# VinAIResearch/Point-Unet

Hardware: AMD Instinct MI355X
Metric: points_per_sec_forward (higher is better)
Workload: dtype f32

## Files before the change

point-unet_amd/csrc/b3_ops.h:

```cpp
#pragma once

#include <hip/hip_runtime.h>

#include "common.h"
#include "mfma_tile.h"

namespace ps {

__device__ __forceinline__ void b3_split_pair(float x, float y, unsigned& q1, unsigned& q2, unsigned& q3)
{
    const unsigned xu = __float_as_uint(x), yu = __float_as_uint(y);
    const float xr = x - __uint_as_float(xu & 0xffff0000u), yr = y - __uint_as_float(yu & 0xffff0000u);
    const unsigned xru = __float_as_uint(xr), yru = __float_as_uint(yr);
    const float x3 = xr - __uint_as_float(xru & 0xffff0000u), y3 = yr - __uint_as_float(yru & 0xffff0000u);
    q1 = __builtin_amdgcn_perm(yu, xu, 0x07060302u);
    q2 = __builtin_amdgcn_perm(yru, xru, 0x07060302u);
    q3 = __builtin_amdgcn_perm(__float_as_uint(y3), __float_as_uint(x3), 0x07060302u);
}
template <int P>
struct BPlanes {
    uint4 p[P];
};
typedef BPlanes<3> B3Planes;
typedef __bf16 b3_bf16x2 __attribute__((ext_vector_type(2)));
// ... 14 lines not shown
    } else {
        r.p[0].x = b3_rne_pair(lo.x, lo.y);
        r.p[0].y = b3_rne_pair(lo.z, lo.w);
        r.p[0].z = b3_rne_pair(hi.x, hi.y);
        r.p[0].w = b3_rne_pair(hi.z, hi.w);
    }
    return r;
}
template <int P>
__device__ __forceinline__ BPlanes<P> b3_split8(const float (&x)[8])
{
    return b3_split8<P>(make_float4(x[0], x[1], x[2], x[3]), make_float4(x[4], x[5], x[6], x[7]));
}
__device__ __forceinline__ f32x16 b3_mfma(const uint4& a, const uint4& b, f32x16 acc)
{
    return __builtin_amdgcn_mfma_f32_32x32x16_bf16(__builtin_bit_cast(bf16x8, a), __builtin_bit_cast(bf16x8, b), acc, 0, 0, 0);
}
template <int P>
__device__ __forceinline__ f32x16 b3_mfma6(const BPlanes<P>& a, const BPlanes<P>& b, f32x16 acc)
{
    if constexpr (P == 3) {
        acc = b3_mfma(a.p[2], b.p[0], acc);
        acc = b3_mfma(a.p[0], b.p[2], acc);
        acc = b3_mfma(a.p[1], b.p[1], acc);
        acc = b3_mfma(a.p[1], b.p[0], acc);
        acc = b3_mfma(a.p[0], b.p[1], acc);
        acc = b3_mfma(a.p[0], b.p[0], acc);
    } else {
        acc = b3_mfma(a.p[0], b.p[0], acc);
    }
    return acc;
}

inline uint16_t b3_piece_of(float w, int plane)
{
    auto trunc16 = [](float x) {
        uint32_t u;
        __builtin_memcpy(&u, &x, 4);
        u &= 0xffff0000u;
        float r;
        __builtin_memcpy(&r, &u, 4);
        return r;
    };
    volatile float w1 = trunc16(w);
    volatile float r1 = w - w1;
    volatile float w2 = trunc16(r1);
    volatile float w3 = r1 - w2;
    const float pick = plane == 0 ? w1 : (plane == 1 ? w2 : w3);
    uint32_t u;
    __builtin_memcpy(&u, &pick, 4);
    return (uint16_t)(u >> 16);
}

template <int P, bool KMAP>
__device__ __forceinline__ void b3_pack_elem(const PackJob& j, int64_t i)
{
    const int ncb = j.cout / 32;
    const int lane = (int)(i & 63), cb = (int)((i >> 6) % ncb), q = (int)((i >> 6) / ncb);
    const int hl = lane >> 5;
    const float* src = j.w + (int64_t)(32 * cb + (lane & 31)) * j.sn;
    float v[8];
#pragma unroll
    for (int e = 0; e < 8; ++e) {
        const int k = KMAP ? 32 * (q >> 1) + 16 * (q & 1) + 8 * (e >> 2) + 4 * hl + (e & 3) : 16 * q + 8 * hl + e;
        v[e] = src[(int64_t)k * j.sk];
    }
// ... 15 lines not shown
```

point-unet_amd/csrc/common.h:

```cpp
#pragma once

#include <hip/hip_runtime.h>

#include <cstdarg>
#include <cstdint>
#include <cstdio>
#include <cstring>
#include <map>
#include <string>
#include <vector>

#include "../../include/pointseg.h"
#include "../../include/pointseg_train_ops.h"

namespace ps {

void set_error(const char* fmt, ...);

#define PS_HIP(expr)                                                                                  \
    do {                                                                                              \
        hipError_t _e = (expr);                                                                       \
        if (_e != hipSuccess) {                                                                       \
            ps::set_error("%s failed: %s (%s:%d)", #expr, hipGetErrorString(_e), __FILE__, __LINE__); \
            return PS_EHIP;                                                                           \
// ... 90 lines not shown
    bool inv_bucket = true;
    int inv_tile = 4096;
    bool gather_reduce_ordered = true;
    int maxpool_bwd_ordered = 1;
    bool train_act_bf16 = true;
    int train_att_gemm_split = -1;
    bool train_att_gemm = true;
    bool train_att128_fwd_gemm = true;
    bool train_fuse_residual = true;
    bool train_merge_syncbn = true;
    int convbn_max_c = 64;
    int convbn_rect_max = 1 << 30;
    bool wgrad_debug = false;
};
void tuning_from_env(Tuning& t);
}

struct ps_context {
    int device = 0;
    ps::Tuning tune;
    hipStream_t own_stream = nullptr;
    hipStream_t stream = nullptr;
    ps::Arena knn_arena;
    ps::Arena net_arena;
    ps::Arena sample_arena;
    ps::DevBuf stage_in;
    ps::DevBuf stage_out;
    ps::DevBuf red_ws;
    ps::DevBuf wgrad_ws;
    ps::PackCache* pack_cache = nullptr;
    ps::DevBuf ops_ring[4];
    int ops_ring_pos = 0;
    bool att_bf16x3 = true;
    bool train_b3 = true;
    bool conv_w_transposed = false;
    bool att_df_accum = false;
    const int32_t* walk_order = nullptr;
    int64_t walk_order_n = 0;
    bool pool_bwd_overwrite = false;
    bool train_bf16 = false;
    bool train_act_bf16 = false;
    bool mid_lds_attr = false;
    size_t chain_lds_attr = 48 * 1024;
    std::map<const void*, size_t> regchain_lds_attr;
    bool deferred = false;
    int32_t* h_flags = nullptr;
    unsigned pending_mask = 0;
    uint64_t builds = 0;
    uint64_t samples = 0;
    uint64_t volume_samples = 0;
    uint64_t flag_serial[8] = {};
    int flag_kind[8] = {};
    int flag_slot = 0;
    int sticky_rc = 0;
    std::string sticky_msg;
    hipEvent_t flag_ev[8] = {};
    std::vector<char> host_ring[8];
    int ring_pos = 0;
    std::vector<char>& ring_next() { ring_pos = (ring_pos + 1) & 7; return host_ring[ring_pos]; }
    int check_deferred();
    int check_flag_slot(int s);
    int defer_status(const void* d_words, size_t bytes, int kind, uint64_t serial);
    struct PinSlot { void* p = nullptr; size_t cap = 0; hipEvent_t ev = nullptr; bool busy = false; };
    PinSlot pin[16];
    int pin_pos = 0;
    int upload_async(void* dst, const void* src, size_t bytes);
// ... 69 lines not shown
```

point-unet_amd/csrc/context.hip:

```cpp
#include "common.h"
#include "kdtree_build.h"

#include <cstdlib>

namespace ps {

static thread_local char g_err[512] = "";

void set_error(const char* fmt, ...)
{
    va_list ap;
    va_start(ap, fmt);
    vsnprintf(g_err, sizeof g_err, fmt, ap);
    va_end(ap);
}

int DevBuf::reserve(size_t bytes)
{
    if (bytes <= cap) return PS_OK;
    if (p) {
        hipError_t e = hipDeviceSynchronize();
        if (e != hipSuccess) {
            set_error("hipDeviceSynchronize failed: %s", hipGetErrorString(e));
            return PS_EHIP;
// ... 186 lines not shown
    flag("PS_TRAIN_ATT128_FWD_GEMM", t.train_att128_fwd_gemm);
    flag("PS_TRAIN_FUSE_RESIDUAL", t.train_fuse_residual);
    flag("PS_TRAIN_MERGE_SYNCBN", t.train_merge_syncbn);
    if (num("PS_CONVBN_MAX_C", v) && v >= 0 && v <= 4096) t.convbn_max_c = (int)v;
    if (num("PS_CONVBN_RECT_MAX", v) && v >= 0) t.convbn_rect_max = v > (double)(1 << 30) ? 1 << 30 : (int)v;
    t.wgrad_debug = std::getenv("PS_WGRAD_DEBUG") != nullptr;
#else
    (void)t;
#endif
}
}

extern "C" {
const char* ps_version(void) { return "pointseg-hip 0.1 gfx950"; }
int ps_abi_version(void) { return PS_ABI_VERSION; }

int ps_create(int device, ps_context** out)
{
    PS_CHECK(out != nullptr, "ps_create: out is NULL");
    int count = 0;
    PS_HIP(hipGetDeviceCount(&count));
    PS_CHECK(device >= 0 && device < count, "ps_create: device %d out of range (%d devices)", device, count);
    PS_HIP(hipSetDevice(device));
    ps_context* c = new ps_context();
    c->device = device;
    hipError_t e = hipStreamCreateWithFlags(&c->own_stream, hipStreamNonBlocking);
    if (e != hipSuccess) {
        delete c;
        ps::set_error("hipStreamCreate failed: %s", hipGetErrorString(e));
        return PS_EHIP;
    }
    c->stream = c->own_stream;
    ps::tuning_from_env(c->tune);
    *out = c;
    return PS_OK;
}

int ps_destroy(ps_context* c)
{
    if (!c) return PS_OK;
    (void)hipSetDevice(c->device);
    (void)hipStreamSynchronize(c->stream);
    c->knn_arena.buf.release();
    c->net_arena.buf.release();
    c->sample_arena.buf.release();
    c->stage_in.release();
    c->stage_out.release();
    c->red_ws.release();
    c->wgrad_ws.release();
    for (auto& b : c->ops_ring) b.release();
    if (c->h_flags) (void)hipHostFree(c->h_flags);
    for (auto& e : c->flag_ev)
        if (e) (void)hipEventDestroy(e);
    for (auto& s : c->pin) {
        if (s.p) (void)hipHostFree(s.p);
        if (s.ev) (void)hipEventDestroy(s.ev);
    }
    for (hipEvent_t e : c->event_pool) (void)hipEventDestroy(e);
    if (c->own_stream) (void)hipStreamDestroy(c->own_stream);
    delete c;
    return PS_OK;
}

int ps_set_stream(ps_context* c, void* hip_stream)
{
    PS_CHECK(c != nullptr, "ps_set_stream: ctx is NULL");
// ... 94 lines not shown
```

point-unet_amd/csrc/debug_hooks.h:

```cpp
#ifndef POINTSEG_DEBUG_H
#define POINTSEG_DEBUG_H
#include "../../include/pointseg.h"
#ifdef __cplusplus
extern "C" {
#endif
int ps_debug_knn_host(const float* support, const float* queries, int64_t B, int64_t n_support,
                      int64_t n_queries, int64_t K, int32_t* out_idx);
int ps_debug_kdtree_host(const float* support, int64_t n, int32_t* vind, int32_t* nodes, float* pts,
                         int32_t* root_depth, float* bbox);
int ps_debug_kdtree_device(ps_context* ctx, const float* support, int64_t n, int32_t* vind, int32_t* nodes,
                           float* pts, int32_t* root_depth, float* bbox);
#define PS_DEBUG_KDTREE_STATS 22
int ps_debug_kdtree_device_set(ps_context* ctx, const float* support, const int32_t* n, int64_t T, const int32_t* want_copy, int32_t* vind,
                               int32_t* nodes, float* pts, int32_t* fat, int32_t* root_depth, float* bbox, float* copy, int32_t* stats);
int ps_debug_pack_weights(const float* W, int cin, int cout, int ntb, float* out);
int ps_debug_pack_b3(const float* W, int cin, int cout, uint16_t* out);
int ps_debug_gemm32(ps_context* ctx, int split_bf16, const float* x1, int ld1, int c1, const int32_t* g1, const float* x2, int ld2, int c2,
                    const int32_t* g2, int gm, int gn, const float* W, const float* bias, int64_t R, int cout, int leaky, float* y, int ldy);
int ps_debug_gemm32_plan(ps_context* ctx, int split_bf16, int64_t R, int cin, int cout, int* out4);

typedef struct ps_debug_chain_layer {
    const float* W;
    const float* bias;
    int cin, cout, leaky;
    float* y;
    int ldy;
    const float* extra;
    int ld_extra, c_extra;
    const int32_t* extra_gather;
} ps_debug_chain_layer;
typedef struct ps_debug_chain_desc {
    int n_layers;
    ps_debug_chain_layer layer[4];
    const float* x1; const int32_t* g1; int ld1, c1, g1m, g1n;
    const float* x2; const int32_t* g2; int ld2, c2, g2m, g2n;
    int64_t R;
} ps_debug_chain_desc;
int ps_debug_chain(ps_context* ctx, const ps_debug_chain_desc* d, int form);
int ps_debug_chain_plan(const ps_debug_chain_desc* d, int* out4);
int ps_debug_att_stage(ps_randla* net, int level, int stage, int form, const float* xyz, const int32_t* idx, const int32_t* order, const float* fg,
                       int64_t n_total, int64_t n_cloud, float* agg);

int ps_debug_set_tuning(ps_context* ctx, const char* field, double value);
int ps_debug_get_tuning(ps_context* ctx, const char* field, double* value);
int ps_debug_tuning_fields(char* buf, int cap);
int ps_debug_volume_sample_args_size(void);

#ifdef __cplusplus
}
#endif
#endif
```

point-unet_amd/csrc/debug_hooks.hip:

```cpp
#include "common.h"

#include <cstring>
#include <vector>
#include "kdtree_build.h"
#include "kdtree_host.h"
#include "rowgemm.h"
#include "attpool.h"
#include "debug_hooks.h"
#include "randla_net.h"

using namespace ps;

extern "C" int ps_debug_volume_sample_args_size(void) { return (int)sizeof(ps_volume_sample_args); }

extern "C" int ps_debug_pack_weights(const float* W, int cin, int cout, int ntb, float* out)
{
    PS_CHECK(W && out && (ntb == 1 || ntb == 2 || ntb == 4), "ps_debug_pack_weights: bad argument");
    pack_weights(W, cin, cout, ntb, out);
    return PS_OK;
}

extern "C" int ps_debug_pack_b3(const float* W, int cin, int cout, uint16_t* out)
{
    PS_CHECK(W && out && cin > 0 && cin % 32 == 0 && cout > 0 && cout % 32 == 0, "ps_debug_pack_b3: bad argument");
// ... 160 lines not shown
        if (form == 0) {
            ChainCache cache;
            if (rowchain_fits(b.steps, b.n, b.s1, b.s2)) rc = rowchain(c, b.steps, b.n, b.s1, b.s2, d->R, &cache);
            else { set_error("ps_debug_chain: the chain fits neither chain kernel (channels above %d, mismatched, or a gathered extra)", kChainMaxC); rc = PS_EINVAL; }
            (void)hipStreamSynchronize(c->stream);
            cache.clear();
        } else if (form == 1) {
            if (regchain_fits(b.steps, b.n, b.s1, b.s2)) rc = regchain(c, b.steps, b.n, b.s1, b.s2, d->R, nullptr);
            else { set_error("ps_debug_chain: not one of regchain's compiled chain shapes"); rc = PS_EINVAL; }
        } else if (form == 2) {
            if (rowchain_lds_plan(b.steps, b.n, b.s1, b.s2, d->R).form == 2) rc = rowchain_lds(c, b.steps, b.n, b.s1, b.s2, d->R);
            else { set_error("ps_debug_chain: the chain does not fit the LDS-staged kernel (channels above %d, mismatched, or a gathered extra)", kChainMaxC); rc = PS_EINVAL; }
        } else {
            RowSrc in1 = b.s1, in2 = b.s2;
            for (int i = 0; i < b.n && rc == PS_OK; ++i) {
                const ChainStep& st = b.steps[i];
                if (i > 0) {
                    in2 = RowSrc();
                    if (st.extra.x) in2 = st.extra;
                }
                float* out = st.y ? st.y : dev + tmp_off[i];
                const int ldo = st.y ? st.ldy : b.L[i].cout;
                rc = rowgemm(c, b.L[i], in1, in2, d->R, out, ldo);
                in1 = RowSrc();
                in1.x = out; in1.ld = ldo; in1.c = b.L[i].cout;
            }
        }
    }
    (void)hipStreamSynchronize(c->stream);
    (void)hipFree(dev);
    return rc;
}

extern "C" int ps_debug_att_stage(ps_randla* net, int level, int stage, int form, const float* xyz, const int32_t* idx, const int32_t* order,
                                  const float* fg, int64_t n_total, int64_t n_cloud, float* agg)
{
    PS_CHECK(net && xyz && idx && fg && agg, "ps_debug_att_stage: NULL argument");
    PS_CHECK(net->have_weights, "ps_debug_att_stage: weights not set");
    PS_CHECK(level >= 0 && level < net->cfg.num_layers && (stage == 1 || stage == 2) && form >= 0 && form <= 3, "ps_debug_att_stage: bad level / stage / form");
    PS_CHECK(n_total >= 0 && n_cloud >= 1 && n_total % n_cloud == 0, "ps_debug_att_stage: n_total must be a whole number of clouds");
    ps_context* c = net->ctx;
    PS_HIP(hipSetDevice(c->device));
    const EncLevel& e = net->enc[level];
    const int d = e.d, h = d / 2;
    const bool use_g = d >= 64;
    AttStage s;
    s.xyz = xyz; s.idx = idx; s.order = order; s.fg = fg; s.lfa1 = &e.lfa1; s.agg = agg;
    s.n_total = n_total; s.n_cloud = n_cloud; s.d = d; s.k = net->cfg.k_n; s.ldf = use_g ? h + d : h;
    s.p32 = e.has_p32 ? &e.p32 : nullptr;
    s.lfa2 = stage == 2 ? &e.lfa2 : nullptr;
    s.wbot = use_g ? (stage == 1 ? &e.bot1 : &e.bot2) : nullptr;
    s.wfull = use_g ? nullptr : (stage == 1 ? &e.full1 : &e.full2);
    int rc = PS_EINVAL;
    if (form == 0) rc = att_pool_stage(c, s);
    else if (form == 1 && att_pool32b_fits(s)) rc = att_pool32b_stage(c, s);
    else if (form == 2 && att_pool32_fits(s)) rc = att_pool32_stage(c, s);
    else if (form == 3) rc = att_pool16_stage(c, s);
    else set_error("ps_debug_att_stage: the level (d = %d, %lld rows) does not fit the 32x32 form %d", d, (long long)n_total, form);
    (void)hipStreamSynchronize(c->stream);
    return rc;
}

static bool is_bool(double v) { return v == 0 || v == 1; }
static bool is_int_in(double v, double lo, double hi) { return v >= lo && v <= hi && v == (double)(int64_t)v; }

#define PS_TUNING_FIELDS(X)                                                \
// ... 176 lines not shown
```

point-unet_amd/csrc/regchain.hip:

```cpp
#include <algorithm>

#include "mfma_tile.h"
#include "rowgemm.h"

namespace ps {

struct RcLayer {
    const float* wp;
    const float* bias;
    float* y;
    const float* ex;
    int ca, cb;
    int ta, tb;
    int cout, ot;
    int ks, ntb;
    int ldy, ldex, leaky;
    int w_off, b_off;
};
struct RcArgs {
    const float* x1; const int32_t* g1; int ld1, g1m, g1n;
    const float* x2; const int32_t* g2; int ld2, g2m, g2n;
    int n, R;
    RcLayer l[kChainMaxSteps];
    const float* image;
    int image_floats;
};

template <int N_, int A0_, int B0_, int O0_, int B1_ = 0, int O1_ = 0, int B2_ = 0, int O2_ = 0, int B3_ = 0, int O3_ = 0>
struct RcShape {
    static constexpr int N = N_, A0 = A0_;
    static constexpr int B[4] = {B0_, B1_, B2_, B3_};
    static constexpr int O[4] = {O0_, O1_, O2_, O3_};
    static constexpr int A(int l) { return l == 0 ? A0_ : O[l - 1]; }
    static constexpr int IN(int l) { return A(l) + B[l]; }
    static constexpr int maxt()
    {
        int m = 1;
        for (int l = 0; l < N_; ++l) {
            m = IN(l) > m ? IN(l) : m;
            m = O[l] > m ? O[l] : m;
        }
        return m;
    }
};

template <int T0, int NT, int MT>
__device__ __forceinline__ void rc_load(float (&dst)[MT][4], const float* __restrict__ rowp, int c, bool vec, int g)
{
#pragma unroll
    for (int t = 0; t < NT; ++t) {
        const int ch = t * 16 + 4 * g;
        if (vec) {
            float4 v = make_float4(0.f, 0.f, 0.f, 0.f);
            if (t + 1 < NT || ch < c) v = *reinterpret_cast<const float4*>(rowp + ch);
            dst[T0 + t][0] = v.x; dst[T0 + t][1] = v.y; dst[T0 + t][2] = v.z; dst[T0 + t][3] = v.w;
        } else {
#pragma unroll
            for (int q = 0; q < 4; ++q) dst[T0 + t][q] = (t + 1 < NT || ch + q < c) ? rowp[ch + q] : 0.f;
        }
    }
}

template <class S, int L>
__device__ __forceinline__ void rc_layer(const RcArgs& a, float (&act)[S::maxt()][4], const float* lds, int lane, int g, int row, int rr, bool ok)
{
    if constexpr (L < S::N) {
        constexpr int IT = S::IN(L), OT = S::O[L], TA = S::A(L), TB = S::B[L];
        const RcLayer& y = a.l[L];
        if constexpr (L > 0 && TB > 0) {
            const bool ve = (y.cb & 3) == 0 && (y.ldex & 3) == 0 && (reinterpret_cast<uintptr_t>(y.ex) & 15) == 0;
            rc_load<TA, TB>(act, y.ex + (size_t)rr * y.ldex, y.cb, ve, g);
        }
        f32x4 acc[OT];
#pragma unroll
        for (int to = 0; to < OT; ++to) acc[to] = f32x4{0.f, 0.f, 0.f, 0.f};
        if constexpr (L > 0) __builtin_amdgcn_sched_barrier(0);
        const float* w = lds + y.w_off + lane;
#pragma unroll
        for (int t0 = 0; t0 < OT; t0 += 4) {
#pragma unroll
            for (int ti = 0; ti < IT; ++ti)
#pragma unroll
                for (int q = 0; q < 4; ++q)
#pragma unroll
                    for (int to = t0; to < (t0 + 4 < OT ? t0 + 4 : OT); ++to)
                        acc[to] = __builtin_amdgcn_mfma_f32_16x16x4f32(w[((to * IT + ti) * 4 + q) * 64], act[ti][q], acc[to], 0, 0, 0);
            if (t0 + 4 < OT) __builtin_amdgcn_sched_barrier(0);
        }
        const bool vy = y.y && (y.cout & 3) == 0 && (y.ldy & 3) == 0 && (reinterpret_cast<uintptr_t>(y.y) & 15) == 0;
#pragma unroll
        for (int to = 0; to < OT; ++to) {
            const int ch = to * 16 + 4 * g;
            const float4 b = *reinterpret_cast<const float4*>(lds + y.b_off + ch);
            float v[4] = {acc[to][0] + b.x, acc[to][1] + b.y, acc[to][2] + b.z, acc[to][3] + b.w};
#pragma unroll
            for (int q = 0; q < 4; ++q) {
                if (y.leaky) v[q] = leaky02(v[q]);
                act[to][q] = v[q];
            }
            if (y.y && ok) {
                float* o = y.y + (size_t)row * y.ldy + ch;
                if (vy) {
                    if (to + 1 < OT || ch < y.cout) *reinterpret_cast<float4*>(o) = make_float4(v[0], v[1], v[2], v[3]);
                } else {
#pragma unroll
                    for (int q = 0; q < 4; ++q)
                        if (to + 1 < OT || ch + q < y.cout) o[q] = v[q];
                }
            }
        }
        rc_layer<S, L + 1>(a, act, lds, lane, g, row, rr, ok);
    }
}

__device__ __forceinline__ void rc_stage(const RcArgs& a, float* dst)
{
    for (int l = 0; l < a.n; ++l) {
        const RcLayer& y = a.l[l];
        const int it_n = y.ta + y.tb;
        const int ln = threadIdx.x & 63, q = threadIdx.x >> 6;
        const int i = ln & 15, gg = ln >> 4;
        const int npairs = it_n * y.ot;
        for (int base = 0; base < npairs; base += 8) {
            float v[8];
#pragma unroll
            for (int u = 0; u < 8; ++u) {
                const int pr = base + u;
                v[u] = 0.f;
                if (pr < npairs) {
                    const int ti = pr / y.ot, to = pr - ti * y.ot;
                    int k;
                    bool kok;
                    if (ti < y.ta) { k = ti * 16 + 4 * gg + q; kok = k < y.ca; }
                    else { k = (ti - y.ta) * 16 + 4 * gg + q; kok = k < y.cb; k += y.ca; }
                    const int cblk = to / y.ntb, j = to - cblk * y.ntb;
                    if (kok && to * 16 + i < y.cout) v[u] = y.wp[(((size_t)cblk * y.ks + (k >> 2)) * 64 + ((k & 3) * 16 + i)) * y.ntb + j];
                }
            }
#pragma unroll
            for (int u = 0; u < 8; ++u) {
                const int pr = base + u;
                if (pr < npairs) {
                    const int ti = pr / y.ot, to = pr - ti * y.ot;
                    dst[y.w_off + ((to * it_n + ti) * 4 + q) * 64 + ln] = v[u];
                }
            }
        }
        for (int e = threadIdx.x; e < y.ot * 16; e += 256) dst[y.b_off + e] = e < y.cout ? y.bias[e] : 0.f;
    }
}

__global__ __launch_bounds__(256) void rc_pack_kernel(RcArgs a, float* out) { rc_stage(a, out); }

template <class S>
__global__ __launch_bounds__(256) void regchain_kernel(RcArgs a)
{
    extern __shared__ __attribute__((aligned(16))) float rc_lds[];
    constexpr int MT = S::maxt();
    const int wave = threadIdx.x >> 6, lane = threadIdx.x & 63;
    const int p = lane & 15, g = lane >> 4;
    if (a.image) {
        for (int i = threadIdx.x; i < a.image_floats / 4; i += 256) reinterpret_cast<float4*>(rc_lds)[i] = reinterpret_cast<const float4*>(a.image)[i];
    } else {
        rc_stage(a, rc_lds);
    }
    __syncthreads();

    const bool v1 = (a.l[0].ca & 3) == 0 && (a.ld1 & 3) == 0 && (reinterpret_cast<uintptr_t>(a.x1) & 15) == 0;
    const bool v2 = (a.l[0].cb & 3) == 0 && (a.ld2 & 3) == 0 && (reinterpret_cast<uintptr_t>(a.x2) & 15) == 0;
    const int stride = gridDim.x * 4;
    auto load_inputs = [&](int tile, float (&dst)[MT][4]) {
        const int rr = min(tile * 16 + p, a.R - 1);
        const int s1 = a.g1 ? (a.g1m ? (rr / a.g1m) * a.g1n : 0) + a.g1[rr] : rr;
        rc_load<0, S::A0>(dst, a.x1 + (size_t)s1 * a.ld1, a.l[0].ca, v1, g);
        if constexpr (S::B[0] > 0) {
            const int s2 = a.g2 ? (a.g2m ? (rr / a.g2m) * a.g2n : 0) + a.g2[rr] : rr;
            rc_load<S::A0, S::B[0]>(dst, a.x2 + (size_t)s2 * a.ld2, a.l[0].cb, v2, g);
        }
    };
    int tile = blockIdx.x * 4 + wave;
    float act[MT][4], nxt[MT][4];
    if (tile * 16 < a.R) load_inputs(tile, nxt);
    for (; tile * 16 < a.R; tile += stride) {
#pragma unroll
        for (int t = 0; t < S::IN(0); ++t)
#pragma unroll
            for (int q = 0; q < 4; ++q) act[t][q] = nxt[t][q];
        if ((tile + stride) * 16 < a.R) load_inputs(tile + stride, nxt);
        const int row = tile * 16 + p;
        rc_layer<S, 0>(a, act, rc_lds, lane, g, row, min(row, a.R - 1), row < a.R);
    }
}

static inline int rc_tiles(int c) { return (c + 15) / 16; }

using RcFc0 = RcShape<2, 1, 0, 1, 0, 1>;
using RcEnc0 = RcShape<2, 1, 0, 1, 1, 2>;
using RcOne0 = RcShape<1, 1, 0, 1>;
using RcPair1 = RcShape<2, 2, 0, 2, 0, 4>;
using RcPair1b = RcShape<2, 4, 0, 2, 0, 4>;
using RcEnc1 = RcShape<2, 4, 0, 4, 2, 8>;
using RcPair2 = RcShape<2, 8, 0, 4, 0, 8>;
using RcHead = RcShape<4, 2, 2, 2, 0, 4, 0, 2, 0, 1>;

template <class S>
static bool rc_matches(const RcArgs& a)
{
    if (a.n != S::N) return false;
    for (int l = 0; l < S::N; ++l)
        if (a.l[l].ta != S::A(l) || a.l[l].tb != S::B[l] || a.l[l].ot != S::O[l]) return false;
    return true;
}

static bool rc_build(const ChainStep* steps, int n_steps, const RowSrc& s1, const RowSrc& s2, RcArgs& a, size_t& lds_bytes)
{
    if (n_steps < 1 || n_steps > kChainMaxSteps) return false;
    a = RcArgs{};
    a.x1 = s1.x; a.g1 = s1.gather; a.ld1 = s1.ld; a.g1m = s1.gm; a.g1n = s1.gn;
    a.x2 = s2.x; a.g2 = s2.gather; a.ld2 = s2.ld; a.g2m = s2.gm; a.g2n = s2.gn;
    a.n = n_steps;
    int off = 0, prev = 0;
    for (int i = 0; i < n_steps; ++i) {
        const PackedLinear* L = steps[i].L;
        if (!L || !L->wp || !L->bias) return false;
        if (steps[i].extra.x && (i == 0 || steps[i].extra.gather)) return false;
        RcLayer& y = a.l[i];
        y.wp = L->wp; y.bias = L->bias; y.y = steps[i].y; y.ldy = steps[i].ldy;
        y.ex = i > 0 ? steps[i].extra.x : nullptr; y.ldex = steps[i].extra.ld;
        y.ca = i == 0 ? s1.c : prev;
        y.cb = i == 0 ? s2.c : (steps[i].extra.x ? steps[i].extra.c : 0);
        if (y.ca + y.cb != L->cin) return false;
        y.ta = rc_tiles(y.ca); y.tb = rc_tiles(y.cb);
        y.cout = L->cout; y.ot = rc_tiles(L->cout);
        y.ks = L->ks; y.ntb = L->ntb; y.leaky = L->leaky;
        y.w_off = off; off += y.ot * (y.ta + y.tb) * 256;
        y.b_off = off; off += y.ot * 16;
        prev = L->cout;
    }
    lds_bytes = (size_t)off * sizeof(float);
    return rc_matches<RcFc0>(a) || rc_matches<RcEnc0>(a) || rc_matches<RcOne0>(a) || rc_matches<RcPair1>(a) || rc_matches<RcPair1b>(a) ||
           rc_matches<RcEnc1>(a) || rc_matches<RcPair2>(a) || rc_matches<RcHead>(a);
}

bool regchain_fits(const ChainStep* steps, int n_steps, const RowSrc& s1, const RowSrc& s2)
{
    RcArgs a;
    size_t lds = 0;
    return rc_build(steps, n_steps, s1, s2, a, lds);
}

static int rc_blocks(int64_t R, size_t lds_bytes)
{
    const int64_t tiles = (R + 15) / 16;
    const int per_cu = std::max(1, std::min(4, (int)(160 * 1024 / std::max<size_t>(lds_bytes, 1))));
    return (int)std::max<int64_t>(1, std::min<int64_t>((tiles + 3) / 4, 256 * per_cu));
}

ChainPlan regchain_plan(const ChainStep* steps, int n_steps, const RowSrc& s1, const RowSrc& s2, int64_t R)
{
    ChainPlan p;
    RcArgs a;
    if (!rc_build(steps, n_steps, s1, s2, a, p.lds_bytes)) return ChainPlan();
    p.form = 1;
    p.blocks = rc_blocks(R, p.lds_bytes);
    return p;
}

template <class S>
static int rc_launch(ps_context* c, const RcArgs& a, size_t lds_bytes, int blocks)
{
    size_t& have = c->regchain_lds_attr[reinterpret_cast<const void*>(regchain_kernel<S>)];
    if (lds_bytes > 48 * 1024 && lds_bytes > have) {
        PS_HIP(hipFuncSetAttribute(reinterpret_cast<const void*>(regchain_kernel<S>), hipFuncAttributeMaxDynamicSharedMemorySize, (int)lds_bytes));
        have = lds_bytes;
    }
    hipLaunchKernelGGL(regchain_kernel<S>, dim3(blocks), dim3(256), lds_bytes, c->stream, a);
    return PS_OK;
}

int regchain(ps_context* c, const ChainStep* steps, int n_steps, const RowSrc& s1, const RowSrc& s2, int64_t R, ChainCache* cache)
{
    if (R <= 0) return PS_OK;
    RcArgs a;
    size_t lds_bytes = 0;
    PS_CHECK(rc_build(steps, n_steps, s1, s2, a, lds_bytes), "regchain: not one of the compiled chain shapes");
    PS_CHECK(R < (int64_t)1 << 31, "regchain: too many rows");
    a.R = (int)R;
    if (cache) {
        ChainCache::Entry* hit = nullptr;
        for (auto& e : cache->entries)
            if (e.wp0 == a.l[0].wp && e.wp_last == a.l[n_steps - 1].wp && e.n == n_steps && e.ca == a.l[0].ca && e.cb == a.l[0].cb) hit = &e;
        if (!hit) {
            cache->entries.emplace_back();
            hit = &cache->entries.back();
            hit->wp0 = a.l[0].wp; hit->wp_last = a.l[n_steps - 1].wp; hit->n = n_steps; hit->ca = a.l[0].ca; hit->cb = a.l[0].cb;
            PS_TRY(hit->img.reserve(lds_bytes));
            hipLaunchKernelGGL(rc_pack_kernel, dim3(1), dim3(256), 0, c->stream, a, hit->img.as<float>());
            PS_HIP(hipGetLastError());
        }
        a.image = hit->img.as<float>();
        a.image_floats = (int)(lds_bytes / sizeof(float));
    }
    const int blocks = rc_blocks(R, lds_bytes);
    if (rc_matches<RcFc0>(a)) PS_TRY(rc_launch<RcFc0>(c, a, lds_bytes, blocks));
    else if (rc_matches<RcEnc0>(a)) PS_TRY(rc_launch<RcEnc0>(c, a, lds_bytes, blocks));
    else if (rc_matches<RcOne0>(a)) PS_TRY(rc_launch<RcOne0>(c, a, lds_bytes, blocks));
    else if (rc_matches<RcPair1>(a)) PS_TRY(rc_launch<RcPair1>(c, a, lds_bytes, blocks));
    else if (rc_matches<RcPair1b>(a)) PS_TRY(rc_launch<RcPair1b>(c, a, lds_bytes, blocks));
    else if (rc_matches<RcEnc1>(a)) PS_TRY(rc_launch<RcEnc1>(c, a, lds_bytes, blocks));
    else if (rc_matches<RcPair2>(a)) PS_TRY(rc_launch<RcPair2>(c, a, lds_bytes, blocks));
    else PS_TRY(rc_launch<RcHead>(c, a, lds_bytes, blocks));
    PS_HIP(hipGetLastError());
    return PS_OK;
}

}
```

point-unet_amd/csrc/rowgemm.h:

```cpp
#pragma once

#include <vector>

#include "common.h"

namespace ps {

struct PackedLinear {
    const float* wp = nullptr;
    const float* wq = nullptr;
    const void* wb = nullptr;
    const float* w32 = nullptr;
    const void* w32b = nullptr;
    const float* bias = nullptr;
    int cin = 0, cout = 0;
    int ks = 0;
    int ntb = 0;
    int cblocks = 0;
    int leaky = 0;
    int accum = 0;
    size_t packed_floats() const { return (size_t)cblocks * ks * 64 * ntb; }
    int nchunks() const { return (cin + 63) / 64; }
    size_t kperm_floats() const { return (size_t)cblocks * nchunks() * 16 * 64 * ntb; }
    size_t bf16_bytes() const { return (size_t)cblocks * nchunks() * 2 * 64 * ntb * 16; }
// ... 8 lines not shown
struct RowSrc {
    const float* x = nullptr;
    const int32_t* gather = nullptr;
    int ld = 0;
    int c = 0;
    int gm = 0, gn = 0;
};

struct Gemm32Plan {
    int rw = 1, cw = 1, sk = 1, pd = 2;
    int rgroups = 0, cgroups = 0;
};
Gemm32Plan gemm32_plan(const Tuning& tn, int64_t R, int cin, int cout);
Gemm32Plan gemm32b_plan(const Tuning& tn, int64_t R, int cin, int cout);
bool gemm32_fits(const PackedLinear& L, const RowSrc& s1, const RowSrc& s2, int64_t R, int ldy);
int gemm32(ps_context* c, const PackedLinear& L, const RowSrc& s1, const RowSrc& s2, int64_t R, float* y, int ldy);
void pack_p32b(const float* W, int cin, int cout, uint16_t* out);
bool gemm32b_fits(const PackedLinear& L, const RowSrc& s1, const RowSrc& s2, int64_t R, int ldy);
int gemm32b(ps_context* c, const PackedLinear& L, const RowSrc& s1, const RowSrc& s2, int64_t R, float* y, int ldy);

int rowgemm(ps_context* c, const PackedLinear& L, const RowSrc& s1, const RowSrc& s2, int64_t R, float* y, int ldy);

constexpr int kChainMaxC = 96;
constexpr int kChainMaxSteps = 4;
struct ChainStep {
    const PackedLinear* L = nullptr;
    float* y = nullptr;
    int ldy = 0;
    RowSrc extra;
};
bool rowchain_fits(const ChainStep* steps, int n_steps, const RowSrc& s1, const RowSrc& s2);
bool regchain_fits(const ChainStep* steps, int n_steps, const RowSrc& s1, const RowSrc& s2);
struct ChainCache {
    struct Entry { const float* wp0 = nullptr; const float* wp_last = nullptr; int n = 0, ca = 0, cb = 0; DevBuf img; };
    std::vector<Entry> entries;
    void clear()
    {
        for (auto& e : entries) e.img.release();
        entries.clear();
    }
};
int regchain(ps_context* c, const ChainStep* steps, int n_steps, const RowSrc& s1, const RowSrc& s2, int64_t R, ChainCache* cache);
int rowchain_lds(ps_context* c, const ChainStep* steps, int n_steps, const RowSrc& s1, const RowSrc& s2, int64_t R);
struct ChainPlan {
    int form = 0;
    int blocks = 0;
    size_t lds_bytes = 0;
    int fast_in = 0;
};
ChainPlan regchain_plan(const ChainStep* steps, int n_steps, const RowSrc& s1, const RowSrc& s2, int64_t R);
ChainPlan rowchain_lds_plan(const ChainStep* steps, int n_steps, const RowSrc& s1, const RowSrc& s2, int64_t R);
ChainPlan rowchain_plan(const ChainStep* steps, int n_steps, const RowSrc& s1, const RowSrc& s2, int64_t R);
int rowchain(ps_context* c, const ChainStep* steps, int n_steps, const RowSrc& s1, const RowSrc& s2, int64_t R, ChainCache* cache = nullptr);

bool gemm_b3_fits(const Tuning& tn, int64_t R, int64_t K, int64_t N, const float* x, int64_t ldx, bool one_plane);
size_t gemm_b3_plane_bytes(int64_t K, int64_t N);
int gemm_b3(ps_context* c, const float* x, int64_t ldx, const float* w, int64_t sk, int64_t sn, const float* bias, int64_t R, int64_t K, int64_t N, int leaky,
            int accumulate, float* y, int64_t ldy, void* planes, int pack = 1);

}
```

Measured before the change: 190.1 million.

## Route selected register-chain shapes through split-bf16x3 MFMA with 512-thread blocks

Adds a second register-chain compute policy that splits fp32 activations and weights into three bf16 planes and accumulates six 16x16x32 bf16 MFMAs per k-pair. The f32 16x16x4 MFMA path is replaced for the Head, Enc1, Pair1 and Pair1b chain shapes, and the new policy runs with 512 threads per block. Weights are pre-split into planes in the LDS image, which makes that image larger. The aim is to use the higher bf16 matrix throughput while keeping roughly fp32 accuracy, at the cost of more LDS per block and extra split arithmetic on activations inside each layer.

```diff
diff --git a/point-unet_amd/csrc/b3_ops.h b/point-unet_amd/csrc/b3_ops.h
--- a/point-unet_amd/csrc/b3_ops.h
+++ b/point-unet_amd/csrc/b3_ops.h
@@ -70,6 +70,21 @@
     return acc;
 }
 
+__device__ __forceinline__ f32x4 b3_mfma16(const uint4& a, const uint4& b, f32x4 acc)
+{
+    return __builtin_amdgcn_mfma_f32_16x16x32_bf16(__builtin_bit_cast(bf16x8, a), __builtin_bit_cast(bf16x8, b), acc, 0, 0, 0);
+}
+__device__ __forceinline__ f32x4 b3_mfma16_6(const B3Planes& a, const B3Planes& b, f32x4 acc)
+{
+    acc = b3_mfma16(a.p[2], b.p[0], acc);
+    acc = b3_mfma16(a.p[0], b.p[2], acc);
+    acc = b3_mfma16(a.p[1], b.p[1], acc);
+    acc = b3_mfma16(a.p[1], b.p[0], acc);
+    acc = b3_mfma16(a.p[0], b.p[1], acc);
+    acc = b3_mfma16(a.p[0], b.p[0], acc);
+    return acc;
+}
+
 inline uint16_t b3_piece_of(float w, int plane)
 {
     auto trunc16 = [](float x) {
diff --git a/point-unet_amd/csrc/common.h b/point-unet_amd/csrc/common.h
--- a/point-unet_amd/csrc/common.h
+++ b/point-unet_amd/csrc/common.h
@@ -146,6 +146,7 @@
     ps::DevBuf ops_ring[4];
     int ops_ring_pos = 0;
     bool att_bf16x3 = true;
+    bool regchain_b3 = true;
     bool train_b3 = true;
     bool conv_w_transposed = false;
     bool att_df_accum = false;
diff --git a/point-unet_amd/csrc/context.hip b/point-unet_amd/csrc/context.hip
--- a/point-unet_amd/csrc/context.hip
+++ b/point-unet_amd/csrc/context.hip
@@ -242,6 +242,9 @@
     }
     c->stream = c->own_stream;
     ps::tuning_from_env(c->tune);
+#ifdef PS_TUNING_ENV
+    if (const char* v = std::getenv("PS_REGCHAIN_B3")) c->regchain_b3 = std::atof(v) != 0;
+#endif
     *out = c;
     return PS_OK;
 }
diff --git a/point-unet_amd/csrc/debug_hooks.h b/point-unet_amd/csrc/debug_hooks.h
--- a/point-unet_amd/csrc/debug_hooks.h
+++ b/point-unet_amd/csrc/debug_hooks.h
@@ -38,6 +38,7 @@
 } ps_debug_chain_desc;
 int ps_debug_chain(ps_context* ctx, const ps_debug_chain_desc* d, int form);
 int ps_debug_chain_plan(const ps_debug_chain_desc* d, int* out4);
+int ps_debug_set_regchain_b3(ps_context* ctx, int on);
 int ps_debug_att_stage(ps_randla* net, int level, int stage, int form, const float* xyz, const int32_t* idx, const int32_t* order, const float* fg,
                        int64_t n_total, int64_t n_cloud, float* agg);
 
diff --git a/point-unet_amd/csrc/debug_hooks.hip b/point-unet_amd/csrc/debug_hooks.hip
--- a/point-unet_amd/csrc/debug_hooks.hip
+++ b/point-unet_amd/csrc/debug_hooks.hip
@@ -216,6 +216,13 @@
     return rc;
 }
 
+extern "C" int ps_debug_set_regchain_b3(ps_context* c, int on)
+{
+    PS_CHECK(c && (on == 0 || on == 1), "ps_debug_set_regchain_b3: bad argument");
+    c->regchain_b3 = on != 0;
+    return PS_OK;
+}
+
 extern "C" int ps_debug_att_stage(ps_randla* net, int level, int stage, int form, const float* xyz, const int32_t* idx, const int32_t* order,
                                   const float* fg, int64_t n_total, int64_t n_cloud, float* agg)
 {
diff --git a/point-unet_amd/csrc/regchain.hip b/point-unet_amd/csrc/regchain.hip
--- a/point-unet_amd/csrc/regchain.hip
+++ b/point-unet_amd/csrc/regchain.hip
@@ -1,5 +1,7 @@
 #include <algorithm>
-
+#include <type_traits>
+
+#include "b3_ops.h"
 #include "mfma_tile.h"
 #include "rowgemm.h"
 
@@ -61,21 +63,13 @@
     }
 }
 
-template <class S, int L>
-__device__ __forceinline__ void rc_layer(const RcArgs& a, float (&act)[S::maxt()][4], const float* lds, int lane, int g, int row, int rr, bool ok)
-{
-    if constexpr (L < S::N) {
-        constexpr int IT = S::IN(L), OT = S::O[L], TA = S::A(L), TB = S::B[L];
-        const RcLayer& y = a.l[L];
-        if constexpr (L > 0 && TB > 0) {
-            const bool ve = (y.cb & 3) == 0 && (y.ldex & 3) == 0 && (reinterpret_cast<uintptr_t>(y.ex) & 15) == 0;
-            rc_load<TA, TB>(act, y.ex + (size_t)rr * y.ldex, y.cb, ve, g);
-        }
-        f32x4 acc[OT];
-#pragma unroll
-        for (int to = 0; to < OT; ++to) acc[to] = f32x4{0.f, 0.f, 0.f, 0.f};
-        if constexpr (L > 0) __builtin_amdgcn_sched_barrier(0);
-        const float* w = lds + y.w_off + lane;
+struct RcF32 {
+    static constexpr int kThreads = 256;
+    static constexpr int kPairFloats = 256;
+    template <int IT, int OT, int MT>
+    static __device__ __forceinline__ void mma(f32x4 (&acc)[OT], const float (&act)[MT][4], const float* wl, int lane)
+    {
+        const float* w = wl + lane;
 #pragma unroll
         for (int t0 = 0; t0 < OT; t0 += 4) {
 #pragma unroll
@@ -87,36 +81,9 @@
                         acc[to] = __builtin_amdgcn_mfma_f32_16x16x4f32(w[((to * IT + ti) * 4 + q) * 64], act[ti][q], acc[to], 0, 0, 0);
             if (t0 + 4 < OT) __builtin_amdgcn_sched_barrier(0);
         }
-        const bool vy = y.y && (y.cout & 3) == 0 && (y.ldy & 3) == 0 && (reinterpret_cast<uintptr_t>(y.y) & 15) == 0;
-#pragma unroll
-        for (int to = 0; to < OT; ++to) {
-            const int ch = to * 16 + 4 * g;
-            const float4 b = *reinterpret_cast<const float4*>(lds + y.b_off + ch);
-            float v[4] = {acc[to][0] + b.x, acc[to][1] + b.y, acc[to][2] + b.z, acc[to][3] + b.w};
-#pragma unroll
-            for (int q = 0; q < 4; ++q) {
-                if (y.leaky) v[q] = leaky02(v[q]);
-                act[to][q] = v[q];
-            }
-            if (y.y && ok) {
-                float* o = y.y + (size_t)row * y.ldy + ch;
-                if (vy) {
-                    if (to + 1 < OT || ch < y.cout) *reinterpret_cast<float4*>(o) = make_float4(v[0], v[1], v[2], v[3]);
-                } else {
-#pragma unroll
-                    for (int q = 0; q < 4; ++q)
-                        if (to + 1 < OT || ch + q < y.cout) o[q] = v[q];
-                }
-            }
-        }
-        rc_layer<S, L + 1>(a, act, lds, lane, g, row, rr, ok);
-    }
-}
-
-__device__ __forceinline__ void rc_stage(const RcArgs& a, float* dst)
-{
-    for (int l = 0; l < a.n; ++l) {
-        const RcLayer& y = a.l[l];
+    }
+    static __device__ __forceinline__ void stage(const RcLayer& y, float* dst)
+    {
         const int it_n = y.ta + y.tb;
         const int ln = threadIdx.x & 63, q = threadIdx.x >> 6;
         const int i = ln & 15, gg = ln >> 4;
@@ -146,29 +113,135 @@
                 }
             }
         }
-        for (int e = threadIdx.x; e < y.ot * 16; e += 256) dst[y.b_off + e] = e < y.cout ? y.bias[e] : 0.f;
-    }
-}
-
-__global__ __launch_bounds__(256) void rc_pack_kernel(RcArgs a, float* out) { rc_stage(a, out); }
-
-template <class S>
-__global__ __launch_bounds__(256) void regchain_kernel(RcArgs a)
+    }
+};
+
+struct RcB3 {
+    static constexpr int kThreads = 512;
+    static constexpr int kPairFloats = 384;
+    template <int IT, int OT, int MT>
+    static __device__ __forceinline__ void mma(f32x4 (&acc)[OT], const float (&act)[MT][4], const float* wl, int lane)
+    {
+        static_assert(IT % 2 == 0, "a k-step of the split-bf16 policy is a pair of 16-channel tiles");
+        constexpr int KP = IT / 2;
+        const uint4* w = reinterpret_cast<const uint4*>(wl) + lane;
+        B3Planes b[KP];
+#pragma unroll
+        for (int kp = 0; kp < KP; ++kp)
+            b[kp] = b3_split8<3>(make_float4(act[2 * kp][0], act[2 * kp][1], act[2 * kp][2], act[2 * kp][3]),
+                                 make_float4(act[2 * kp + 1][0], act[2 * kp + 1][1], act[2 * kp + 1][2], act[2 * kp + 1][3]));
+#pragma unroll
+        for (int t0 = 0; t0 < OT; t0 += 4) {
+#pragma unroll
+            for (int kp = 0; kp < KP; ++kp)
+#pragma unroll
+                for (int to = t0; to < (t0 + 4 < OT ? t0 + 4 : OT); ++to) {
+                    B3Planes a;
+#pragma unroll
+                    for (int pl = 0; pl < 3; ++pl) a.p[pl] = w[((to * KP + kp) * 3 + pl) * 64];
+                    acc[to] = b3_mfma16_6(a, b[kp], acc[to]);
+                }
+            if (t0 + 4 < OT) __builtin_amdgcn_sched_barrier(0);
+        }
+    }
+    static __device__ __forceinline__ void stage(const RcLayer& y, float* dst)
+    {
+        const int kp_n = (y.ta + y.tb) / 2;
+        uint4* out = reinterpret_cast<uint4*>(dst + y.w_off);
+        for (int s = threadIdx.x; s < y.ot * kp_n * 64; s += kThreads) {
+            const int ln = s & 63, slot = s >> 6;
+            const int to = slot / kp_n, kp = slot - to * kp_n;
+            const int i = ln & 15, gg = ln >> 4;
+            const int cblk = to / y.ntb, j = to - cblk * y.ntb;
+            float v[8];
+#pragma unroll
+            for (int e = 0; e < 8; ++e) {
+                const int ti = 2 * kp + (e >> 2), q = e & 3;
+                int k;
+                bool kok;
+                if (ti < y.ta) { k = ti * 16 + 4 * gg + q; kok = k < y.ca; }
+                else { k = (ti - y.ta) * 16 + 4 * gg + q; kok = k < y.cb; k += y.ca; }
+                v[e] = 0.f;
+                if (kok && to * 16 + i < y.cout) v[e] = y.wp[(((size_t)cblk * y.ks + (k >> 2)) * 64 + ((k & 3) * 16 + i)) * y.ntb + j];
+            }
+            const B3Planes p = b3_split8<3>(v);
+#pragma unroll
+            for (int pl = 0; pl < 3; ++pl) out[(slot * 3 + pl) * 64 + ln] = p.p[pl];
+        }
+    }
+};
+
+template <class S, class P, int L>
+__device__ __forceinline__ void rc_layer(const RcArgs& a, float (&act)[S::maxt()][4], const float* lds, int lane, int g, int row, int rr, bool ok)
+{
+    if constexpr (L < S::N) {
+        constexpr int IT = S::IN(L), OT = S::O[L], TA = S::A(L), TB = S::B[L];
+        const RcLayer& y = a.l[L];
+        if constexpr (L > 0 && TB > 0) {
+            const bool ve = (y.cb & 3) == 0 && (y.ldex & 3) == 0 && (reinterpret_cast<uintptr_t>(y.ex) & 15) == 0;
+            rc_load<TA, TB>(act, y.ex + (size_t)rr * y.ldex, y.cb, ve, g);
+        }
+        f32x4 acc[OT];
+#pragma unroll
+        for (int to = 0; to < OT; ++to) acc[to] = f32x4{0.f, 0.f, 0.f, 0.f};
+        if constexpr (L > 0) __builtin_amdgcn_sched_barrier(0);
+        P::template mma<IT, OT>(acc, act, lds + y.w_off, lane);
+        const bool vy = y.y && (y.cout & 3) == 0 && (y.ldy & 3) == 0 && (reinterpret_cast<uintptr_t>(y.y) & 15) == 0;
+#pragma unroll
+        for (int to = 0; to < OT; ++to) {
+            const int ch = to * 16 + 4 * g;
+            const float4 b = *reinterpret_cast<const float4*>(lds + y.b_off + ch);
+            float v[4] = {acc[to][0] + b.x, acc[to][1] + b.y, acc[to][2] + b.z, acc[to][3] + b.w};
+#pragma unroll
+            for (int q = 0; q < 4; ++q) {
+                if (y.leaky) v[q] = leaky02(v[q]);
+                act[to][q] = v[q];
+            }
+            if (y.y && ok) {
+                float* o = y.y + (size_t)row * y.ldy + ch;
+                if (vy) {
+                    if (to + 1 < OT || ch < y.cout) *reinterpret_cast<float4*>(o) = make_float4(v[0], v[1], v[2], v[3]);
+                } else {
+#pragma unroll
+                    for (int q = 0; q < 4; ++q)
+                        if (to + 1 < OT || ch + q < y.cout) o[q] = v[q];
+                }
+            }
+        }
+        rc_layer<S, P, L + 1>(a, act, lds, lane, g, row, rr, ok);
+    }
+}
+
+template <class P>
+__device__ __forceinline__ void rc_stage(const RcArgs& a, float* dst)
+{
+    for (int l = 0; l < a.n; ++l) {
+        const RcLayer& y = a.l[l];
+        P::stage(y, dst);
+        for (int e = threadIdx.x; e < y.ot * 16; e += P::kThreads) dst[y.b_off + e] = e < y.cout ? y.bias[e] : 0.f;
+    }
+}
+
+template <class P>
+__global__ __launch_bounds__(P::kThreads) void rc_pack_kernel(RcArgs a, float* out) { rc_stage<P>(a, out); }
+
+template <class S, class P>
+__global__ __launch_bounds__(P::kThreads) void regchain_kernel(RcArgs a)
 {
     extern __shared__ __attribute__((aligned(16))) float rc_lds[];
-    constexpr int MT = S::maxt();
+    constexpr int MT = S::maxt(), WAVES = P::kThreads / 64;
     const int wave = threadIdx.x >> 6, lane = threadIdx.x & 63;
     const int p = lane & 15, g = lane >> 4;
     if (a.image) {
-        for (int i = threadIdx.x; i < a.image_floats / 4; i += 256) reinterpret_cast<float4*>(rc_lds)[i] = reinterpret_cast<const float4*>(a.image)[i];
+        for (int i = threadIdx.x; i < a.image_floats / 4; i += P::kThreads) reinterpret_cast<float4*>(rc_lds)[i] = reinterpret_cast<const float4*>(a.image)[i];
     } else {
-        rc_stage(a, rc_lds);
+        rc_stage<P>(a, rc_lds);
     }
     __syncthreads();
 
     const bool v1 = (a.l[0].ca & 3) == 0 && (a.ld1 & 3) == 0 && (reinterpret_cast<uintptr_t>(a.x1) & 15) == 0;
     const bool v2 = (a.l[0].cb & 3) == 0 && (a.ld2 & 3) == 0 && (reinterpret_cast<uintptr_t>(a.x2) & 15) == 0;
-    const int stride = gridDim.x * 4;
+    const int stride = gridDim.x * WAVES;
     auto load_inputs = [&](int tile, float (&dst)[MT][4]) {
         const int rr = min(tile * 16 + p, a.R - 1);
         const int s1 = a.g1 ? (a.g1m ? (rr / a.g1m) * a.g1n : 0) + a.g1[rr] : rr;
@@ -178,7 +251,7 @@
             rc_load<S::A0, S::B[0]>(dst, a.x2 + (size_t)s2 * a.ld2, a.l[0].cb, v2, g);
         }
     };
-    int tile = blockIdx.x * 4 + wave;
+    int tile = blockIdx.x * WAVES + wave;
     float act[MT][4], nxt[MT][4];
     if (tile * 16 < a.R) load_inputs(tile, nxt);
     for (; tile * 16 < a.R; tile += stride) {
@@ -188,7 +261,7 @@
             for (int q = 0; q < 4; ++q) act[t][q] = nxt[t][q];
         if ((tile + stride) * 16 < a.R) load_inputs(tile + stride, nxt);
         const int row = tile * 16 + p;
-        rc_layer<S, 0>(a, act, rc_lds, lane, g, row, min(row, a.R - 1), row < a.R);
+        rc_layer<S, P, 0>(a, act, rc_lds, lane, g, row, min(row, a.R - 1), row < a.R);
     }
 }
 
@@ -212,6 +285,28 @@
     return true;
 }
 
+template <class S>
+constexpr bool rc_even_inputs()
+{
+    for (int l = 0; l < S::N; ++l)
+        if (S::IN(l) & 1) return false;
+    return true;
+}
+template <class S>
+constexpr bool kRcSplit = std::is_same<S, RcHead>::value || std::is_same<S, RcEnc1>::value || std::is_same<S, RcPair1>::value ||
+                          std::is_same<S, RcPair1b>::value;
+
+static size_t rc_layout(RcArgs& a, int pair_floats)
+{
+    int off = 0;
+    for (int i = 0; i < a.n; ++i) {
+        RcLayer& y = a.l[i];
+        y.w_off = off; off += y.ot * (y.ta + y.tb) * pair_floats;
+        y.b_off = off; off += y.ot * 16;
+    }
+    return (size_t)off * sizeof(float);
+}
+
 static bool rc_build(const ChainStep* steps, int n_steps, const RowSrc& s1, const RowSrc& s2, RcArgs& a, size_t& lds_bytes)
 {
     if (n_steps < 1 || n_steps > kChainMaxSteps) return false;
@@ -219,7 +314,7 @@
     a.x1 = s1.x; a.g1 = s1.gather; a.ld1 = s1.ld; a.g1m = s1.gm; a.g1n = s1.gn;
     a.x2 = s2.x; a.g2 = s2.gather; a.ld2 = s2.ld; a.g2m = s2.gm; a.g2n = s2.gn;
     a.n = n_steps;
-    int off = 0, prev = 0;
+    int prev = 0;
     for (int i = 0; i < n_steps; ++i) {
         const PackedLinear* L = steps[i].L;
         if (!L || !L->wp || !L->bias) return false;
@@ -233,11 +328,9 @@
         y.ta = rc_tiles(y.ca); y.tb = rc_tiles(y.cb);
         y.cout = L->cout; y.ot = rc_tiles(L->cout);
         y.ks = L->ks; y.ntb = L->ntb; y.leaky = L->leaky;
-        y.w_off = off; off += y.ot * (y.ta + y.tb) * 256;
-        y.b_off = off; off += y.ot * 16;
         prev = L->cout;
     }
-    lds_bytes = (size_t)off * sizeof(float);
+    lds_bytes = rc_layout(a, RcF32::kPairFloats);
     return rc_matches<RcFc0>(a) || rc_matches<RcEnc0>(a) || rc_matches<RcOne0>(a) || rc_matches<RcPair1>(a) || rc_matches<RcPair1b>(a) ||
            rc_matches<RcEnc1>(a) || rc_matches<RcPair2>(a) || rc_matches<RcHead>(a);
 }
@@ -249,11 +342,11 @@
     return rc_build(steps, n_steps, s1, s2, a, lds);
 }
 
-static int rc_blocks(int64_t R, size_t lds_bytes)
+static int rc_blocks(int64_t R, size_t lds_bytes, int waves)
 {
     const int64_t tiles = (R + 15) / 16;
-    const int per_cu = std::max(1, std::min(4, (int)(160 * 1024 / std::max<size_t>(lds_bytes, 1))));
-    return (int)std::max<int64_t>(1, std::min<int64_t>((tiles + 3) / 4, 256 * per_cu));
+    const int per_cu = std::max(1, std::min(16 / waves, (int)(160 * 1024 / std::max<size_t>(lds_bytes, 1))));
+    return (int)std::max<int64_t>(1, std::min<int64_t>((tiles + waves - 1) / waves, 256 * per_cu));
 }
 
 ChainPlan regchain_plan(const ChainStep* steps, int n_steps, const RowSrc& s1, const RowSrc& s2, int64_t R)
@@ -262,20 +355,48 @@
     RcArgs a;
     if (!rc_build(steps, n_steps, s1, s2, a, p.lds_bytes)) return ChainPlan();
     p.form = 1;
-    p.blocks = rc_blocks(R, p.lds_bytes);
+    p.blocks = rc_blocks(R, p.lds_bytes, RcF32::kThreads / 64);
     return p;
 }
 
+template <class S, class P>
+static int rc_run(ps_context* c, RcArgs& a, ChainCache* cache)
+{
+    constexpr bool split = std::is_same<P, RcB3>::value;
+    const size_t lds_bytes = rc_layout(a, P::kPairFloats);
+    if (cache) {
+        ChainCache::Entry* hit = nullptr;
+        for (auto& e : cache->entries)
+            if (e.wp0 == a.l[0].wp && e.wp_last == a.l[a.n - 1].wp && e.n == a.n && e.ca == a.l[0].ca && e.cb == a.l[0].cb && e.split == split) hit = &e;
+        if (!hit) {
+            cache->entries.emplace_back();
+            hit = &cache->entries.back();
+            hit->wp0 = a.l[0].wp; hit->wp_last = a.l[a.n - 1].wp; hit->n = a.n; hit->ca = a.l[0].ca; hit->cb = a.l[0].cb; hit->split = split;
+            PS_TRY(hit->img.reserve(lds_bytes));
+            hipLaunchKernelGGL(rc_pack_kernel<P>, dim3(1), dim3(P::kThreads), 0, c->stream, a, hit->img.as<float>());
+            PS_HIP(hipGetLastError());
+        }
+        a.image = hit->img.as<float>();
+        a.image_floats = (int)(lds_bytes / sizeof(float));
+    }
+    size_t& have = c->regchain_lds_attr[reinterpret_cast<const void*>(regchain_kernel<S, P>)];
+    if (lds_bytes > 48 * 1024 && lds_bytes > have) {
+        PS_HIP(hipFuncSetAttribute(reinterpret_cast<const void*>(regchain_kernel<S, P>), hipFuncAttributeMaxDynamicSharedMemorySize, (int)lds_bytes));
+        have = lds_bytes;
+    }
+    hipLaunchKernelGGL((regchain_kernel<S, P>), dim3(rc_blocks(a.R, lds_bytes, P::kThreads / 64)), dim3(P::kThreads), lds_bytes, c->stream, a);
+    PS_HIP(hipGetLastError());
+    return PS_OK;
+}
+
 template <class S>
-static int rc_launch(ps_context* c, const RcArgs& a, size_t lds_bytes, int blocks)
-{
-    size_t& have = c->regchain_lds_attr[reinterpret_cast<const void*>(regchain_kernel<S>)];
-    if (lds_bytes > 48 * 1024 && lds_bytes > have) {
-        PS_HIP(hipFuncSetAttribute(reinterpret_cast<const void*>(regchain_kernel<S>), hipFuncAttributeMaxDynamicSharedMemorySize, (int)lds_bytes));
-        have = lds_bytes;
-    }
-    hipLaunchKernelGGL(regchain_kernel<S>, dim3(blocks), dim3(256), lds_bytes, c->stream, a);
-    return PS_OK;
+static int rc_route(ps_context* c, RcArgs& a, ChainCache* cache)
+{
+    if constexpr (kRcSplit<S>) {
+        static_assert(rc_even_inputs<S>(), "the split-bf16 policy takes its K axis in pairs of 16-channel tiles");
+        if (c->regchain_b3) return rc_run<S, RcB3>(c, a, cache);
+    }
+    return rc_run<S, RcF32>(c, a, cache);
 }
 
 int regchain(ps_context* c, const ChainStep* steps, int n_steps, const RowSrc& s1, const RowSrc& s2, int64_t R, ChainCache* cache)
@@ -286,32 +407,14 @@
     PS_CHECK(rc_build(steps, n_steps, s1, s2, a, lds_bytes), "regchain: not one of the compiled chain shapes");
     PS_CHECK(R < (int64_t)1 << 31, "regchain: too many rows");
     a.R = (int)R;
-    if (cache) {
-        ChainCache::Entry* hit = nullptr;
-        for (auto& e : cache->entries)
-            if (e.wp0 == a.l[0].wp && e.wp_last == a.l[n_steps - 1].wp && e.n == n_steps && e.ca == a.l[0].ca && e.cb == a.l[0].cb) hit = &e;
-        if (!hit) {
-            cache->entries.emplace_back();
-            hit = &cache->entries.back();
-            hit->wp0 = a.l[0].wp; hit->wp_last = a.l[n_steps - 1].wp; hit->n = n_steps; hit->ca = a.l[0].ca; hit->cb = a.l[0].cb;
-            PS_TRY(hit->img.reserve(lds_bytes));
-            hipLaunchKernelGGL(rc_pack_kernel, dim3(1), dim3(256), 0, c->stream, a, hit->img.as<float>());
-            PS_HIP(hipGetLastError());
-        }
-        a.image = hit->img.as<float>();
-        a.image_floats = (int)(lds_bytes / sizeof(float));
-    }
-    const int blocks = rc_blocks(R, lds_bytes);
-    if (rc_matches<RcFc0>(a)) PS_TRY(rc_launch<RcFc0>(c, a, lds_bytes, blocks));
-    else if (rc_matches<RcEnc0>(a)) PS_TRY(rc_launch<RcEnc0>(c, a, lds_bytes, blocks));
-    else if (rc_matches<RcOne0>(a)) PS_TRY(rc_launch<RcOne0>(c, a, lds_bytes, blocks));
-    else if (rc_matches<RcPair1>(a)) PS_TRY(rc_launch<RcPair1>(c, a, lds_bytes, blocks));
-    else if (rc_matches<RcPair1b>(a)) PS_TRY(rc_launch<RcPair1b>(c, a, lds_bytes, blocks));
-    else if (rc_matches<RcEnc1>(a)) PS_TRY(rc_launch<RcEnc1>(c, a, lds_bytes, blocks));
-    else if (rc_matches<RcPair2>(a)) PS_TRY(rc_launch<RcPair2>(c, a, lds_bytes, blocks));
-    else PS_TRY(rc_launch<RcHead>(c, a, lds_bytes, blocks));
-    PS_HIP(hipGetLastError());
-    return PS_OK;
-}
-
-}
+    if (rc_matches<RcFc0>(a)) return rc_route<RcFc0>(c, a, cache);
+    if (rc_matches<RcEnc0>(a)) return rc_route<RcEnc0>(c, a, cache);
+    if (rc_matches<RcOne0>(a)) return rc_route<RcOne0>(c, a, cache);
+    if (rc_matches<RcPair1>(a)) return rc_route<RcPair1>(c, a, cache);
+    if (rc_matches<RcPair1b>(a)) return rc_route<RcPair1b>(c, a, cache);
+    if (rc_matches<RcEnc1>(a)) return rc_route<RcEnc1>(c, a, cache);
+    if (rc_matches<RcPair2>(a)) return rc_route<RcPair2>(c, a, cache);
+    return rc_route<RcHead>(c, a, cache);
+}
+
+}
diff --git a/point-unet_amd/csrc/rowgemm.h b/point-unet_amd/csrc/rowgemm.h
--- a/point-unet_amd/csrc/rowgemm.h
+++ b/point-unet_amd/csrc/rowgemm.h
@@ -64,7 +64,7 @@
 bool rowchain_fits(const ChainStep* steps, int n_steps, const RowSrc& s1, const RowSrc& s2);
 bool regchain_fits(const ChainStep* steps, int n_steps, const RowSrc& s1, const RowSrc& s2);
 struct ChainCache {
-    struct Entry { const float* wp0 = nullptr; const float* wp_last = nullptr; int n = 0, ca = 0, cb = 0; DevBuf img; };
+    struct Entry { const float* wp0 = nullptr; const float* wp_last = nullptr; int n = 0, ca = 0, cb = 0; bool split = false; DevBuf img; };
     std::vector<Entry> entries;
     void clear()
     {
```

Result: faster. 192.6 million (median of 6 runs) (+1.3%).
